# jeffreychou777/GenComm

Measured on AMD Instinct MI355X. Metric: scenes/sec, higher is better.
Workload: dtype f32

## Files before the change

### gencomm_amd/csrc/gencomm_abi.hip

```cpp
#include "../../include/gencomm_hip.h"

#include "common.h"
#include "conv_kernels.h"
#include "detect_kernels.h"
#include "enhancer_host.h"
#include "fusion_kernels.h"
#include "msgext_host.h"
#include "noise_kernels.h"
#include "pillar_kernels.h"
#include "pfn_kernels.h"
#include "train_kernels.h"
#include "wgrad_h3_kernels.h"
#include "unet_bwd_host.h"
#include "unet_host.h"

#include <algorithm>
#include <atomic>
#include <map>
#include <mutex>
#include <string>
#include <stdlib.h>
#include <string.h>

namespace gc {
// ... 470 lines not shown
  if (const char* e = w.build(p, n, H, W)) return fail(GC_ERR_ARG, e);
  if ((long long)w.total > workspace_bytes) return fail(GC_ERR_WORKSPACE, "workspace too small (see gencomm_denoise_workspace_bytes)");
  hipStream_t st = (hipStream_t)stream;
  const bool philox = noise0 == nullptr;
  const long long per_agent = (long long)C * H * W;

  UNetCall c{&p, &w, prepared, (char*)workspace, n, H, W, st, modes_snapshot()};
  if (int rc = check_bf16_mode(c.m, p, W)) return rc;
  GC_HIP(hipMemsetAsync(c.amax(), 0, 256, st));
  amax_kernel<<<256, 256, 0, st>>>(cond, (long long)n * 2 * H * W, c.amax());
  QSampleArgs q{feat, src_row, noise0, sched + (size_t)(T - 1) * 5, out, seed, (unsigned)T, per_agent, seed_dev, c.amax() + 1};
  launch_q_sample(q, n, philox, st);

  const long long smode = c.m.v[MODE_SAMPLER];
  const bool want_latent = smode == 2 || (smode == 0 && pick_tile(c.m, n, H, W) == TILE_64x16);
  const bool latent = want_latent && T >= 2 && (W % 4) == 0;
  if (!latent) {
    for (int i = 0; i < T; ++i) {
      const int t = T - 1 - i;
      ConvOutArgs co{};
      co.out = out;
      co.xt = out;
      co.sched = sched + (size_t)t * 5;
      co.noise = philox ? nullptr : step_noise + (size_t)i * n * per_agent;
      co.seed = seed;
      co.seed_dev = seed_dev;
      co.stream_id = (unsigned)t;
      const int post = t == 0 ? 0 : (philox ? 2 : 1);
      if (int rc = unet_enqueue(c, out, cond, t, post, co)) return rc;
    }
    return GC_OK;
  }
  const int nops = (int)p.ops.size();
  kmap_enqueue(c, cond);
  for (int i = 0; i < T; ++i) {
    const int t = T - 1 - i;
    ConvOutArgs co{};
    co.out = out;
    if (int rc = unet_enqueue_range(c, out, cond, t, 0, co, i == 0 ? 0 : 1, t == 0 ? nops : nops - 1, i != 0, i == 0)) return rc;
    if (t > 0) {
      const float* nz = philox ? nullptr : step_noise + (size_t)i * n * per_agent;
      if (int rc = latent_step_enqueue(c, sched + (size_t)t * 5, nz, seed, (unsigned)t, seed_dev)) return rc;
    }
  }
  return GC_OK;
}

int gencomm_enhancer_num_params(int C) {
  EnhancerPlan p;
  if (const char* e = p.build(C)) { fail(GC_ERR_ARG, e); return -1; }
  return (int)p.params.size();
}
int gencomm_enhancer_param_info(int C, int index, char* name, int name_cap, long long* numel, long long* offset) {
  EnhancerPlan p;
  if (const char* e = p.build(C)) return fail(GC_ERR_ARG, e);
  GC_CHECK_ARG(index >= 0 && index < (int)p.params.size(), "param index out of range");
  GC_CHECK_ARG(name && name_cap > 0 && numel && offset, "null output pointer");
  snprintf(name, (size_t)name_cap, "%s", p.params[index].name.c_str());
  *numel = p.params[index].numel;
  *offset = p.params[index].off;
  return GC_OK;
}
long long gencomm_enhancer_raw_floats(int C) {
  EnhancerPlan p;
  if (const char* e = p.build(C)) { fail(GC_ERR_ARG, e); return -1; }
  return p.raw_floats;
}
long long gencomm_enhancer_workspace_bytes(int n, int C, int H, int W) {
  EnhancerPlan p;
  if (const char* e = p.build(C)) { fail(GC_ERR_ARG, e); return -1; }
  if (n < 1 || H < 1 || W < 1) { fail(GC_ERR_ARG, "n, H, W must be positive"); return -1; }
  return (long long)enhancer_workspace_bytes(p, n, H, W);
// ... 614 lines not shown
```

### gencomm_amd/csrc/latent_kernels.h

```cpp
#pragma once
#include "unet_kernels.h"

namespace gc {

struct PrepLatentArgs {
  const float* w_in;
  const float* w_out;
  const float* b_out;
  float* wc5; float* wc1; float* bring; float* bsum;
  int C;
};
__global__ void prep_latent_kernel(const PrepLatentArgs a) {
  const int idx = blockIdx.x * blockDim.x + threadIdx.x;
  const int C = a.C, CI = C + 2;
  auto Wx = [&](int o, int c, int t) { return (double)a.w_in[((size_t)o * CI + 2 + c) * 9 + t]; };
  auto Wo = [&](int c, int i, int t) { return (double)a.w_out[((size_t)c * 8 + i) * 9 + t]; };
  if (idx < 1600) {
    const int o = idx & 7, d = (idx >> 3) % 25, i = idx / 200;
    const int dy = d / 5, dx = d % 5;
    double s = 0.0;
    for (int t1y = 0; t1y < 3; ++t1y)
      for (int t1x = 0; t1x < 3; ++t1x) {
        const int t2y = dy - t1y, t2x = dx - t1x;
        if (t2y < 0 || t2y > 2 || t2x < 0 || t2x > 2) continue;
// ... 10 lines not shown
    const int j = idx - 1600 - 5184, o = j & 7, t1 = j >> 3;
    double s = 0.0;
    for (int c = 0; c < C; ++c) s += Wx(o, c, t1) * (double)a.b_out[c];
    a.bring[j] = (float)s;
  } else if (idx < 1600 + 5184 + 72 + 8) {
    const int o = idx - 1600 - 5184 - 72;
    double s = 0.0;
    for (int t1 = 0; t1 < 9; ++t1)
      for (int c = 0; c < C; ++c) s += Wx(o, c, t1) * (double)a.b_out[c];
    a.bsum[o] = (float)s;
  }
}

struct LatentArgs {
  const float* a_src;
  const double* a_stat;
  const float* gamma; const float* beta;
  const float* kmap;
  float* hs0;
  double* hs0_stat;
  const float* wc5; const float* wc1; const float* bring; const float* bsum;
  const float* wx;
  const float* wc5h;
  const float* wxh;
  const float* noise;
  const float* sched;
  double inv_cnt;
  unsigned long long seed;
  unsigned int stream_id;
  int C, H, W;
  const unsigned long long* seed_dev;
  int xcd;
  int a_bf16;
};

template <int TW, int TH, int NOISE>
__global__ __launch_bounds__((TW / 4) * TH) void latent_step_kernel(const LatentArgs a) {
  constexpr int NT = (TW / 4) * TH, QPR = TW / 4;
  constexpr int LH5 = TH + 4, LH = TH + 2, LS = TW + 8;
  static_assert(NT / QPR == TH, "one staging pass must cover TH rows");
  __shared__ __align__(16) float smem[8 * LH5 * LS];
  __shared__ float s_ab[8][2];
  __shared__ float s_red[NT / 64][16];
  float (*tileA)[LH5][LS] = reinterpret_cast<float (*)[LH5][LS]>(smem);
  float (*tileE)[LH][LS] = reinterpret_cast<float (*)[LH][LS]>(smem);

  const int tid = threadIdx.x, lane = tid & 63;
  const BlockId bid = xcd_block(a.xcd);
  const int n = bid.z;
  const int x0 = bid.x * TW, y0 = bid.y * TH;
  const int tx = tid % QPR, ty = tid / QPR;
  const int H = a.H, W = a.W;
  const unsigned plane = (unsigned)(H * W);
  const float c1 = as_const(a.sched)[2], c2 = as_const(a.sched)[3], sg = as_const(a.sched)[4];
  const unsigned long long seed = (NOISE == 2 && a.seed_dev) ? *a.seed_dev : a.seed;

  float wc[25];
  load_wregs<25>(wc, a.wc5, 1600, lane);
  const float* __restrict__ ap = a.a_src + (size_t)n * 8 * plane;
  float4 qm[8], qr[(4 * 8 * QPR + NT - 1) / NT];
  constexpr int NREM = (4 * 8 * QPR + NT - 1) / NT;
  constexpr int NHAL = (8 * LH5 * 4 + NT - 1) / NT;
  float hh[NHAL];
  auto load_quad = [&](int c, int r, int qx) {
    const int gy = y0 - 2 + r, gx = x0 + 4 * qx;
    float4 v = make_float4(0.f, 0.f, 0.f, 0.f);
    if (r < LH5 && gy >= 0 && gy < H && gx < W) v = *reinterpret_cast<const float4*>(ap + ((unsigned)c * plane + (unsigned)gy * (unsigned)W + (unsigned)gx));
    return v;
  };
#pragma unroll
  for (int c = 0; c < 8; ++c) qm[c] = load_quad(c, ty, tx);
#pragma unroll
  for (int j = 0; j < NREM; ++j) {
    const int idx = tid + j * NT;
    const int c = idx / (4 * QPR), rr = TH + (idx / QPR) % 4;
    qr[j] = c < 8 ? load_quad(c, rr, tx) : make_float4(0.f, 0.f, 0.f, 0.f);
  }
#pragma unroll
  for (int j = 0; j < NHAL; ++j) {
// ... 231 lines not shown
```

### gencomm_amd/csrc/latenth_kernels.h

```cpp
#pragma once
#include "conv8b_kernels.h"
#include "conv8h_kernels.h"
#include "latent_kernels.h"

namespace gc {

constexpr int HL_LH5 = HC_TH + 4;
constexpr int HL_PLANE5 = HL_LH5 * HC_ROW;
constexpr int HL_W5TAB3 = 8 * HC_WC3;
constexpr int HL_TPLANE5 = HL_PLANE5 / 2;
constexpr int HL_RING = (2 * (HC_TW + 4) + 2 * HL_LH5) * 8;

__global__ __launch_bounds__(256) void prep_latent_h_kernel(const float* __restrict__ wc5, const float* __restrict__ w_in ,
                                                           float* __restrict__ dst5, float* __restrict__ dstx,
                                                           float* __restrict__ dstc, int C) {
  __shared__ float s_max[256];
  const int tid = threadIdx.x;
  const int CI = C + 2;
  float m = 0.f;
  for (int i = tid; i < 1600; i += 256) m = fmaxf(m, fabsf(wc5[i]));
  for (int i = tid; i < 8 * CI * 9; i += 256) m = fmaxf(m, fabsf(w_in[i]));
  s_max[tid] = m;
  __syncthreads();
  for (int s = 128; s > 0; s >>= 1) {
// ... 103 lines not shown
      const float* __restrict__ w = a.wc1 + (t1 * 9 + t2) * 64;
#pragma unroll 2
      for (int i = 0; i < 8; ++i) {
        float av[4];
#pragma unroll
        for (int p = 0; p < 4; ++p) {
          const int tr = trow + t1y + t2y, tp = px0 + p + t1x + t2x - 2;
          av[p] = inp[p] ? ring[hl_ring_slot(y0 - 2 + tr, x0 + tp, tr, tp, H, W) * 8 + i] : 0.f;
        }
#pragma unroll
        for (int o = 0; o < 4; ++o) {
          const float wv = w[i * 8 + oc0 + o] * sc;
#pragma unroll
          for (int p = 0; p < 4; ++p) accp[p][o] = fmaf(-wv, av[p], accp[p][o]);
        }
      }
    }
  }
}


struct ConvInHArgs {
  const float* cond;
  const float* x;
  const float* wch;
  const float* wxh;
  const float* scales;
  const float* bias;
  float* dst;
  double* dstat;
  int C, H, W;
  int xcd;
  const float* amax;
};

__global__ __launch_bounds__(HC_NT, 3) void conv_in_h_kernel(const ConvInHArgs a) {
  constexpr int NT = HC_NT, TW = HC_TW, TH = HC_TH;
  __shared__ __align__(16) unsigned char tile[2 * HC_PLANE + HC_TPLANE];
  __shared__ float s_red[NT / 64][16];
  fp16_ovfl_clamp();
  const int tid = threadIdx.x, lane = tid & 63, wave = tid >> 6;
  const BlockId bid = xcd_block(a.xcd);
  const int n = bid.z;
  const int x0 = bid.x * TW, y0 = bid.y * TH;
  const int H = a.H, W = a.W;
  const unsigned plane = (unsigned)(H * W);
  const int ln = lane & 15, g = lane >> 4, ch = g & 1, rr = g >> 1;
  const int gx = x0 + 4 * ln, gy0 = y0 + 4 * wave + rr;
  const bool wave_live = y0 + 4 * wave < H;
  const int r0 = tid >> 4, qx = tid & 15;
  const float mul = a.amax != nullptr ? act_scale(fmaxf(a.amax[0], a.C > 0 ? a.amax[1] : 0.f)) : 1.0f;
  const float inv_s = a.scales[0] / mul, sc = a.scales[1] * mul;

  f32x4 acc[2][4];
  {
    const float4 b4 = *reinterpret_cast<const float4*>(a.bias + 4 * ch);
    const f32x4 b0 = {b4.x * sc, b4.y * sc, b4.z * sc, b4.w * sc};
#pragma unroll
    for (int p = 0; p < 2; ++p)
#pragma unroll
      for (int j = 0; j < 4; ++j) acc[p][j] = b0;
  }
  int off[4][3];
  hc_lane_offsets(off, wave, lane);
  const int nchunk = a.C / 8;
  const float* __restrict__ xp = a.x + (size_t)n * a.C * plane;
  TileRegs<TW, TH, NT, 8> R;
  float2 hreg = make_float2(0.f, 0.f);
  {
    const float* __restrict__ sp = a.cond + (size_t)n * 2 * plane;
    TileRegs<TW, TH, NT, 2> Rc;
    stage_load<TW, TH, NT, 2, false>(Rc, sp, plane, W, H, W, x0, y0, tid);
    float2 hc = make_float2(0.f, 0.f);
    if (tid < HC_LH * 8 && (tid & 3) == 0) {
      const int side = (tid >> 2) & 1, r = tid >> 3;
      const int gy = y0 - 1 + r, gxh = side ? x0 + TW : x0 - 1;
      if (gy >= 0 && gy < H && gxh >= 0 && gxh < W) {
        hc.x = sp[(unsigned)gy * (unsigned)W + (unsigned)gxh];
        hc.y = sp[plane + (unsigned)gy * (unsigned)W + (unsigned)gxh];
      }
    }
    if (nchunk > 0) {
      stage_load<TW, TH, NT, 8, false>(R, xp, plane, W, H, W, x0, y0, tid);
      hreg = halo_load_h<false>(xp, plane, W, H, W, x0, y0, tid);
    }
    float e[8][4];
#pragma unroll
    for (int c = 0; c < 8; ++c)
#pragma unroll
      for (int j = 0; j < 4; ++j) e[c][j] = 0.f;
    e[0][0] = Rc.v[0].x * mul; e[0][1] = Rc.v[0].y * mul; e[0][2] = Rc.v[0].z * mul; e[0][3] = Rc.v[0].w * mul;
    e[1][0] = Rc.v[1].x * mul; e[1][1] = Rc.v[1].y * mul; e[1][2] = Rc.v[1].z * mul; e[1][3] = Rc.v[1].w * mul;
    hc_store_main3(tile, r0, qx, e);
    const float er[4] = {Rc.vr.x * mul, Rc.vr.y * mul, Rc.vr.z * mul, Rc.vr.w * mul};
    hc_store_rem3(tile, tid, er);
    if (tid < HC_LH * 8) hc_store_halo3(tile, tid, hc.x * mul, hc.y * mul);
    __syncthreads();
    if (wave_live) conv_tile_mfma3<false, true>(tile, a.wch, acc, off, lane);
  }
#pragma unroll 1
  for (int cc = 0; cc < nchunk; ++cc) {
    __syncthreads();
    stage_store_h<false, true>(tile, R, hreg, H, W, x0, y0, nullptr, tid, mul);
    if (cc + 1 < nchunk) {
      stage_load<TW, TH, NT, 8, false>(R, xp + (size_t)(cc + 1) * 8 * plane, plane, W, H, W, x0, y0, tid);
      hreg = halo_load_h<false>(xp + (size_t)(cc + 1) * 8 * plane, plane, W, H, W, x0, y0, tid);
    }
    __syncthreads();
    if (wave_live) conv_tile_mfma3<false, true>(tile, a.wxh + (size_t)cc * HC_WTAB3, acc, off, lane);
  }

  float part[8];
#pragma unroll
  for (int i = 0; i < 8; ++i) part[i] = 0.f;
  if (wave_live) {
#pragma unroll
    for (int p = 0; p < 2; ++p) {
      const int gy = gy0 + 2 * p;
      if (gy < H && gx + 3 < W) {
#pragma unroll
        for (int i = 0; i < 4; ++i) {
          float v[4];
#pragma unroll
          for (int j = 0; j < 4; ++j) {
            v[j] = acc[p][j][i] * inv_s;
            part[i] += v[j];
            part[4 + i] = fmaf(v[j], v[j], part[4 + i]);
          }
          *reinterpret_cast<float4*>(a.dst + ((size_t)n * 8 + 4 * ch + i) * plane + (size_t)gy * W + gx) = make_float4(v[0], v[1], v[2], v[3]);
        }
      }
// ... 163 lines not shown
            if (POST != 0) {
              const float4 t4 = *reinterpret_cast<const float4*>(a.xt + e);
              const float xt[4] = {t4.x, t4.y, t4.z, t4.w};
              if (POST == 1) {
                const float4 z4 = *reinterpret_cast<const float4*>(a.noise + e);
                const float z[4] = {z4.x, z4.y, z4.z, z4.w};
#pragma unroll
                for (int j = 0; j < 4; ++j) v[j] = fmaf(sg, z[j], fmaf(c1, v[j], c2 * xt[j]));
              } else {
#pragma unroll
                for (int j = 0; j < 4; ++j) v[j] = z8[4 * ii + j] + fmaf(c1, v[j], c2 * xt[j]);
              }
            }
            *reinterpret_cast<float4*>(a.out + e) = make_float4(v[0], v[1], v[2], v[3]);
            if (POST != 0) amax = fmaxf(amax, fmaxf(fmaxf(fabsf(v[0]), fabsf(v[1])), fmaxf(fabsf(v[2]), fabsf(v[3]))));
          }
        }
      }
    }
  }
  if (POST != 0 && a.amax_out != nullptr) wave_amax_commit(amax, a.amax_out);
}

template <int NOISE>
__global__ __launch_bounds__(HC_NT, 3) void latent_step_h_kernel(const LatentArgs a) {
  constexpr int NT = HC_NT, TW = HC_TW, TH = HC_TH;
  constexpr int TILE_BYTES = NOISE == 1 ? 2 * HC_PLANE + HC_TPLANE : 2 * HL_PLANE5;
  __shared__ __align__(16) unsigned char tile[TILE_BYTES];
  __shared__ float s_ring[HL_RING];
  __shared__ float s_ab[8][2];
  __shared__ float s_red[NT / 64][16];

  fp16_ovfl_clamp();
  const int tid = threadIdx.x, lane = tid & 63, wave = tid >> 6;
  const BlockId bid = xcd_block(a.xcd);
  const int n = bid.z;
  const int x0 = bid.x * TW, y0 = bid.y * TH;
  const int H = a.H, W = a.W;
  const unsigned plane = (unsigned)(H * W);
  const float c1 = a.sched[2], c2 = a.sched[3], sg = a.sched[4];
  const unsigned long long seed = (NOISE == 2 && a.seed_dev) ? *a.seed_dev : a.seed;
  const int ln = lane & 15, g = lane >> 4, ch = g & 1, rr = g >> 1;
  const int gx = x0 + 4 * ln;
  const int gy0 = y0 + 4 * wave + rr;
  const bool wave_live = y0 + 4 * wave < H;

  const int af32 = !a.a_bf16;
  const size_t abase = (size_t)n * 8 * plane;
  float4 qm[8], qr[2];
  float hh[2][2];
  const int r0 = tid >> 4, qx = tid & 15;
  const bool ok_m = (y0 - 2 + r0) >= 0 && (y0 - 2 + r0) < H && (x0 + 4 * qx) < W;
#pragma unroll
  for (int c = 0; c < 8; ++c)
    qm[c] = ok_m ? ld4(a.a_src, af32, abase + ((unsigned)c * plane + (unsigned)(y0 - 2 + r0) * (unsigned)W + (unsigned)(x0 + 4 * qx)))
                 : make_float4(0.f, 0.f, 0.f, 0.f);
  const int rrow = TH + ((tid & 63) >> 4), cpr = tid >> 6;
  const bool ok_r = (y0 - 2 + rrow) >= 0 && (y0 - 2 + rrow) < H && (x0 + 4 * qx) < W;
#pragma unroll
  for (int k = 0; k < 2; ++k)
    qr[k] = ok_r ? ld4(a.a_src, af32, abase + ((unsigned)(2 * cpr + k) * plane + (unsigned)(y0 - 2 + rrow) * (unsigned)W + (unsigned)(x0 + 4 * qx)))
                 : make_float4(0.f, 0.f, 0.f, 0.f);
  bool ok_h[2];
#pragma unroll
  for (int j = 0; j < 2; ++j) {
    const int idx = tid + j * NT;
// ... 283 lines not shown
```

### gencomm_amd/csrc/unet_host.h

```cpp
#pragma once
#include <stdlib.h>

#include "attn_kernels.h"
#include "conv8b_kernels.h"
#include "conv8h_kernels.h"
#include "conv8h8_kernels.h"
#include "dataflow_kernels.h"
#include "latent_kernels.h"
#include "latenth_kernels.h"
#include "unet_kernels.h"
#include "unet_plan.h"

namespace gc {

inline int cdiv(int a, int b) { return (a + b - 1) / b; }

enum TileCfg { TILE_64x16 = 0, TILE_32x16 = 1, TILE_32x8 = 2 };
inline long long tile_want(const Modes& m) {
  return m.v[MODE_TILE_WANT] > 0 ? m.v[MODE_TILE_WANT] : (m.split() ? 160LL : 512LL);
}
inline TileCfg pick_tile(const Modes& m, int n, int H, int W, int zmul = 1) {
  if (m.bf16()) return TILE_64x16;
  const long long want = tile_want(m);
  if ((long long)cdiv(W, 64) * cdiv(H, 16) * n * zmul >= want) return TILE_64x16;
// ... 51 lines not shown
  }
  GC_KLOG(t == TILE_64x16 ? "conv8_kernel<64,16,4,...> (exact fp32)" : t == TILE_32x16 ? "conv8_kernel<32,16,4,...> (exact fp32)" : "conv8_kernel<32,8,1,...> (exact fp32)");
  switch (t) {
    case TILE_64x16: conv8_kernel<64, 16, 4, NSRC, GN, UP, RES><<<grid, 256, 0, st>>>(a); break;
    case TILE_32x16: conv8_kernel<32, 16, 4, NSRC, GN, UP, RES><<<grid, 128, 0, st>>>(a); break;
    default: conv8_kernel<32, 8, 1, NSRC, GN, UP, RES><<<grid, 256, 0, st>>>(a); break;
  }
}

template <int NSRC, bool GN, bool UP, int RES>
inline void launch_conv8b(const Conv8BArgs& a, int n, hipStream_t st) {
  const double elt = 2.0;
  const double abytes = elt * n * ((double)NSRC * 8 * a.Hin * a.Win + (RES == 1 ? 8.0 : RES == 2 ? 16.0 : 0.0) * a.H * a.W + 8.0 * a.H * a.W);
  TimedLaunch tl(UP ? KF_UP : (NSRC == 2 ? KF_CONV16 : (RES == 1 ? KF_CONV8_RES1 : RES == 2 ? KF_CONV8_RES2 : KF_CONV8)), st, abytes);
  GC_KLOG("conv8b_kernel<...> (bf16 storage)");
  conv8b_kernel<NSRC, GN, UP, RES><<<dim3(cdiv(a.W, 64), cdiv(a.H, 16), n), 256, 0, st>>>(a);
}

struct UNetCall {
  const UNetPlan* plan;
  const UNetWorkspace* ws;
  const float* prepared;
  char* wsp;
  int n, H, W;
  hipStream_t st;
  Modes m;
  float* amax() const { return reinterpret_cast<float*>(wsp + ws->amax_off); }
  int is_f32(int id) const { return (!m.bf16() || id == plan->hs0_tensor) ? 1 : 0; }

  float* tensor_ptr(int id) const {
    const TensorPlan& t = plan->tensors[id];
    return reinterpret_cast<float*>(wsp + ws->level_base[t.level] + ws->slot_bytes[t.level] * t.slot);
  }
  double* stat_ptr(int id) const { return reinterpret_cast<double*>(wsp) + (size_t)id * n * 16; }
};

inline Conv8Args conv1_args(const UNetCall& c, const Op& o, int t) {
  const ResBlockPlan& b = c.plan->blocks[o.blk];
  const float* P = c.prepared;
  const int Hl = c.ws->Hl[o.level], Wl = c.ws->Wl[o.level];
  Conv8Args a{};
  a.src[0] = c.tensor_ptr(o.src[0]); a.sstat[0] = c.stat_ptr(o.src[0]);
  if (o.src[1] >= 0) { a.src[1] = c.tensor_ptr(o.src[1]); a.sstat[1] = c.stat_ptr(o.src[1]); }
  a.gamma = P + b.n1w; a.beta = P + b.n1b;
  a.w = P + b.p_c1w; a.wh = P + b.p_c1wh; a.bias = P + b.p_bias1 + (size_t)t * 8;
  a.dst = c.tensor_ptr(o.dst); a.dstat = c.stat_ptr(o.dst);
  a.H = a.Hin = Hl; a.W = a.Win = Wl;
  a.inv_cnt = 1.0 / ((b.cin == 8 ? 2.0 : 4.0) * Hl * Wl);
  a.xcd = c.m.xcd();
  return a;
}
inline Conv8Args conv2_args(const UNetCall& c, const Op& o) {
  const ResBlockPlan& b = c.plan->blocks[o.blk];
  const float* P = c.prepared;
  const int Hl = c.ws->Hl[o.level], Wl = c.ws->Wl[o.level];
  Conv8Args a{};
  a.src[0] = c.tensor_ptr(o.src[0]); a.sstat[0] = c.stat_ptr(o.src[0]);
  a.gamma = P + b.n2w; a.beta = P + b.n2b;
  a.w = P + b.p_c2w; a.wh = P + b.p_c2wh; a.bias = P + b.p_bias2;
  a.res[0] = c.tensor_ptr(o.res[0]);
  if (o.res[1] >= 0) { a.res[1] = c.tensor_ptr(o.res[1]); a.ninw = P + b.p_ninw; }
  a.dst = c.tensor_ptr(o.dst); a.dstat = c.stat_ptr(o.dst);
  a.H = a.Hin = Hl; a.W = a.Win = Wl;
  a.inv_cnt = 1.0 / (2.0 * Hl * Wl);
  a.xcd = c.m.xcd();
  return a;
}
// ... 4 lines not shown
  Conv8Args a{};
  a.src[0] = c.tensor_ptr(o.src[0]);
  a.sstat[0] = c.stat_ptr(o.src[0]);
  a.w = P + p.up[lin].p_w; a.wh = P + p.up[lin].p_wh; a.bias = P + p.up[lin].b;
  a.dst = c.tensor_ptr(o.dst); a.dstat = c.stat_ptr(o.dst);
  a.H = c.ws->Hl[o.level]; a.W = c.ws->Wl[o.level]; a.Hin = c.ws->Hl[lin]; a.Win = c.ws->Wl[lin];
  a.xcd = c.m.xcd();
  return a;
}
inline DownArgs down_args(const UNetCall& c, const Op& o) {
  const UNetPlan& p = *c.plan;
  const float* P = c.prepared;
  const int lin = o.level - 1;
  return DownArgs{c.tensor_ptr(o.src[0]), P + p.down[lin].p_w, P + p.down[lin].b, c.tensor_ptr(o.dst), c.stat_ptr(o.dst),
                  c.ws->Hl[o.level], c.ws->Wl[o.level], c.ws->Hl[lin], c.ws->Wl[lin], !c.is_f32(o.src[0]), !c.is_f32(o.dst)};
}

inline bool resfuse_emulated(const UNetCall& c, const ResBlockPlan& b, TileCfg tc, bool wvec) {
  return c.m.v[MODE_RESFUSE_EMU] != 0 && b.cin == 8 && tc == TILE_64x16 && c.m.split() && !c.m.bf16() && wvec;
}

inline bool df_eligible(const UNetCall& c, int f, int l) {
  if (c.m.v[MODE_DATAFLOW] == 0 || !c.m.split() || c.m.bf16() || l - f < 2 || l - f > DF_MAX_OPS || c.n > 64 * 1024) return false;
  if (c.m.v[MODE_CONV8H_MASK] != -1) return false;
  for (int oi = f; oi < l; ++oi) {
    const Op& o = c.plan->ops[oi];
    if (o.kind != OP_RES_CONV1 && o.kind != OP_RES_CONV2 && o.kind != OP_DOWN && o.kind != OP_UP) return false;
    if (o.kind == OP_DOWN) {
      if ((c.ws->Wl[o.level - 1] & 3) != 0) return false;
    } else if (pick_tile(c.m, c.n, c.ws->Hl[o.level], c.ws->Wl[o.level]) != TILE_64x16) return false;
  }
  return true;
}
inline int df_enqueue(const UNetCall& c, int t, int f, int l, bool upload) {
  const UNetPlan& p = *c.plan;
  DfProgram* dprog = reinterpret_cast<DfProgram*>(c.wsp + c.ws->df_prog_off);
  unsigned* words = reinterpret_cast<unsigned*>(c.wsp + c.ws->df_words_off);
  const int nops = l - f;
  if (upload) {
    static thread_local DfProgram hp;
    hp.nops = nops; hp.n = c.n;
    int qlen[8] = {0, 0, 0, 0, 0, 0, 0, 0};
    for (int k = 0; k < nops; ++k) {
      const Op& o = p.ops[f + k];
      DfOp& d = hp.ops[k];
      d = DfOp{};
      const int Hl = c.ws->Hl[o.level], Wl = c.ws->Wl[o.level];
      if (o.kind == OP_DOWN) {
        d.kind = DF_DOWN; d.tx = cdiv(Hl * ((Wl + 1) / 2), 256); d.ty = 1; d.down = down_args(c, o);
      } else {
        d.tx = cdiv(Wl, 64); d.ty = cdiv(Hl, 16);
        if (o.kind == OP_RES_CONV1) {
          d.kind = p.blocks[o.blk].cin == 8 ? DF_CONV1 : DF_CONV16; d.conv = conv1_args(c, o, 0); d.bias_stride = 8;
        } else if (o.kind == OP_RES_CONV2) {
          d.kind = p.blocks[o.blk].cin == 8 ? DF_CONV2_RES1 : DF_CONV2_RES2; d.conv = conv2_args(c, o);
        } else {
          d.kind = DF_UP; d.conv = up_args(c, o);
        }
      }
      d.tiles = d.tx * d.ty;
      d.items = d.tiles * c.n;
      const int qq = d.items >> 3, rr = d.items & 7;
      for (int x = 0; x <= 8; ++x) d.item_base[x] = x * qq + (x < rr ? x : rr);
      for (int x = 0; x < 8; ++x) { d.ticket_base[x] = qlen[x]; qlen[x] += d.item_base[x + 1] - d.item_base[x]; }
    }
    for (int x = 0; x < 8; ++x) hp.queue_len[x] = qlen[x];
    for (int k0 = 0; k0 < nops; k0 += DF_CHUNK) {
      DfUploadArgs ua{};
      ua.dst = dprog; ua.first = k0; ua.count = std::min(DF_CHUNK, nops - k0); ua.nops = nops; ua.n = c.n;
      for (int x = 0; x < 8; ++x) ua.queue_len[x] = qlen[x];
      for (int k = 0; k < ua.count; ++k) ua.ops[k] = hp.ops[k0 + k];
      df_upload_kernel<<<1, 64, 0, c.st>>>(ua);
    }
  }
  int dev = 0, cus = 256;
  if (hipGetDevice(&dev) == hipSuccess) (void)hipDeviceGetAttribute(&cus, hipDeviceAttributeMultiprocessorCount, dev);
  DfArgs da{dprog, words, words + 8, words + 8 + 64 * (size_t)c.n, t, c.m.v[MODE_DATAFLOW] == 2 ? 1 : 0};
  GC_KLOG("unet_dataflow_kernel (persistent, per-agent layer dependencies)");
  TimedLaunch tl(KF_DATAFLOW, c.st);
  unet_dataflow_kernel<<<dim3(3 * cus), HC_NT, 0, c.st>>>(da);
  GC_HIP(hipGetLastError());
  return GC_OK;
}

inline int unet_enqueue_range(const UNetCall& c, const float* x_t, const float* cond, int t, int post,
                              ConvOutArgs co, int first, int last, bool keep_hs0_stats, bool df_upload = true) {
  const UNetPlan& p = *c.plan;
  const float* P = c.prepared;
  {
    const size_t skip = keep_hs0_stats ? (size_t)c.n * 16 * sizeof(double) : 0;
    GC_HIP(hipMemsetAsync(c.wsp + skip, 0, c.ws->stats_bytes - skip, c.st));
  }
  const int df_f = std::max(first, 1), df_l = std::min(last, (int)p.ops.size() - 1);
  const bool dataflow = df_eligible(c, df_f, df_l);
  for (int oi = first; oi < last; ++oi) {
    if (dataflow && oi == df_f) {
      if (int rc = df_enqueue(c, t, df_f, df_l, df_upload)) return rc;
      oi = df_l - 1;
      continue;
    }
    const Op& o = p.ops[oi];
    const int Hl = c.ws->Hl[o.level], Wl = c.ws->Wl[o.level];
    switch (o.kind) {
      case OP_CONV_IN: {
        ConvInArgs a{cond, x_t, P + p.conv_in.p_w, P + p.conv_in.b, c.tensor_ptr(o.dst), c.stat_ptr(o.dst), p.C, Hl, Wl, c.m.xcd()};
        const TileCfg tc = pick_tile(c.m, c.n, Hl, Wl);
        int tw, th;
        tile_dims(tc, &tw, &th);
        const dim3 grid(cdiv(Wl, tw), cdiv(Hl, th), c.n);
        TimedLaunch tl(KF_CONV_IN, c.st);
        if (tc == TILE_64x16 && c.m.split() && (Wl & 3) == 0) {
          ConvInHArgs ah{cond, x_t, P + p.p_wch, P + p.p_wxh, P + p.p_wc5h + HL_W5TAB3, P + p.conv_in.b, c.tensor_ptr(o.dst),
                         c.stat_ptr(o.dst), p.C, Hl, Wl, c.m.xcd(), c.amax()};
          GC_KLOG("conv_in_h_kernel");
          conv_in_h_kernel<<<grid, 256, 0, c.st>>>(ah);
        } else {
          GC_KLOG("conv_in_kernel<tile> (exact fp32)");
          if (tc == TILE_64x16) conv_in_kernel<64, 16, 4><<<grid, 256, 0, c.st>>>(a);
          else if (tc == TILE_32x16) conv_in_kernel<32, 16, 4><<<grid, 128, 0, c.st>>>(a);
          else conv_in_kernel<32, 8, 1><<<grid, 256, 0, c.st>>>(a);
        }
        break;
      }
      case OP_RES_CONV1: {
        const ResBlockPlan& b = p.blocks[o.blk];
        if (c.m.bf16()) {
          Conv8BArgs a{};
          a.src[0] = c.tensor_ptr(o.src[0]); a.src_f32[0] = c.is_f32(o.src[0]); a.sstat[0] = c.stat_ptr(o.src[0]);
          if (o.src[1] >= 0) { a.src[1] = c.tensor_ptr(o.src[1]); a.src_f32[1] = c.is_f32(o.src[1]); a.sstat[1] = c.stat_ptr(o.src[1]); }
          a.gamma = P + b.n1w; a.beta = P + b.n1b; a.wb = P + b.p_c1wb; a.bias = P + b.p_bias1 + (size_t)t * 8;
          a.dst = c.tensor_ptr(o.dst); a.dst_f32 = c.is_f32(o.dst); a.dstat = c.stat_ptr(o.dst);
          a.H = a.Hin = Hl; a.W = a.Win = Wl; a.inv_cnt = 1.0 / ((b.cin == 8 ? 2.0 : 4.0) * Hl * Wl); a.xcd = c.m.xcd();
          if (b.cin == 8) launch_conv8b<1, true, false, 0>(a, c.n, c.st);
          else launch_conv8b<2, true, false, 0>(a, c.n, c.st);
          break;
        }
        const Conv8Args a = conv1_args(c, o, t);
        const TileCfg tc = pick_tile(c.m, c.n, Hl, Wl);
        if (resfuse_emulated(c, b, tc, (Wl & 3) == 0)) {
          Conv8Args e = a;
          e.term_mask = 63 | 64;
          TimedLaunch tl(KF_CONV8, c.st, 4.0 * c.n * 8.0 * Hl * Wl);
          GC_KLOG("conv8h_kernel<1,GN,0,0,DIAG> (MODE_RESFUSE_EMU: statistics only)");
          conv8h_kernel<1, true, false, 0, true><<<dim3(cdiv(Wl, 64), cdiv(Hl, 16), c.n), 256, 0, c.st>>>(e);
          break;
        }
// ... 80 lines not shown
        tile_dims(tc, &tw, &th);
        const dim3 grid(cdiv(Wl, tw), cdiv(Hl, th), c.n * nocb);
#define GC_LAUNCH_CO(POST)                                                             \
  do {                                                                                 \
    if (tc == TILE_64x16) conv_out_kernel<64, 16, 4, POST><<<grid, 256, 0, c.st>>>(co); \
    else conv_out_kernel<32, 8, 1, POST><<<grid, 256, 0, c.st>>>(co);                  \
  } while (0)
        TimedLaunch tl(KF_CONV_OUT, c.st);
        if (c.m.split() && (Wl & 3) == 0 && pick_tile(c.m, c.n, Hl, Wl) == TILE_64x16) {
          const dim3 gh(cdiv(Wl, 64), cdiv(Hl, 16), c.n);
          GC_KLOG(post == 0 ? "conv_out_h_kernel<0> (x0_hat)" : post == 1 ? "conv_out_h_kernel<1> (explicit noise)" : "conv_out_h_kernel<2> (in-kernel Philox)");
          if (post == 0) conv_out_h_kernel<0><<<gh, 256, 0, c.st>>>(co);
          else if (post == 1) conv_out_h_kernel<1><<<gh, 256, 0, c.st>>>(co);
          else conv_out_h_kernel<2><<<gh, 256, 0, c.st>>>(co);
        } else {
          GC_KLOG(post == 0 ? "conv_out_kernel<tile,0> (exact fp32, x0_hat)" : post == 1 ? "conv_out_kernel<tile,1> (exact fp32, explicit noise)" : "conv_out_kernel<tile,2> (exact fp32, in-kernel Philox)");
          if (post == 0) GC_LAUNCH_CO(0);
          else if (post == 1) GC_LAUNCH_CO(1);
          else GC_LAUNCH_CO(2);
        }
#undef GC_LAUNCH_CO
        break;
      }
    }
  }
  GC_HIP(hipGetLastError());
  return GC_OK;
}

inline int unet_enqueue(const UNetCall& c, const float* x_t, const float* cond, int t, int post, ConvOutArgs co) {
  return unet_enqueue_range(c, x_t, cond, t, post, co, 0, (int)c.plan->ops.size(), false);
}

inline void kmap_enqueue(const UNetCall& c, const float* cond) {
  const UNetPlan& p = *c.plan;
  ConvInArgs a{cond, nullptr, c.prepared + p.conv_in.p_w, c.prepared + p.conv_in.b,
               reinterpret_cast<float*>(c.wsp + c.ws->kmap_off), nullptr, 0, c.H, c.W, c.m.xcd()};
  const TileCfg tc = pick_tile(c.m, c.n, c.H, c.W);
  int tw, th;
  tile_dims(tc, &tw, &th);
  const dim3 grid(cdiv(c.W, tw), cdiv(c.H, th), c.n);
  if (tc == TILE_64x16 && c.m.split() && (c.W & 3) == 0) {
    ConvInHArgs ah{cond, nullptr, c.prepared + p.p_wch, c.prepared + p.p_wxh, c.prepared + p.p_wc5h + HL_W5TAB3, c.prepared + p.conv_in.b,
                   reinterpret_cast<float*>(c.wsp + c.ws->kmap_off), nullptr, 0, c.H, c.W, c.m.xcd(), c.amax()};
    conv_in_h_kernel<<<grid, 256, 0, c.st>>>(ah);
  } else if (tc == TILE_64x16) conv_in_kernel<64, 16, 4><<<grid, 256, 0, c.st>>>(a);
  else if (tc == TILE_32x16) conv_in_kernel<32, 16, 4><<<grid, 128, 0, c.st>>>(a);
  else conv_in_kernel<32, 8, 1><<<grid, 256, 0, c.st>>>(a);
}

inline int latent_step_enqueue(const UNetCall& c, const float* sched_row, const float* noise, unsigned long long seed,
                               unsigned stream_id, const unsigned long long* seed_dev = nullptr) {
  const UNetPlan& p = *c.plan;
  const float* P = c.prepared;
  GC_HIP(hipMemsetAsync(c.stat_ptr(p.hs0_tensor), 0, (size_t)c.n * 16 * sizeof(double), c.st));
  LatentArgs a{};
  a.a_src = c.tensor_ptr(p.last_body_tensor); a.a_stat = c.stat_ptr(p.last_body_tensor);
  a.gamma = P + p.nout_w; a.beta = P + p.nout_b;
  a.kmap = reinterpret_cast<const float*>(c.wsp + c.ws->kmap_off);
  a.hs0 = c.tensor_ptr(p.hs0_tensor); a.hs0_stat = c.stat_ptr(p.hs0_tensor);
  a.wc5 = P + p.p_wc5; a.wc1 = P + p.p_wc1; a.bring = P + p.p_bring; a.bsum = P + p.p_bsum;
  a.wx = P + p.conv_in.p_w + 144;
  a.wc5h = P + p.p_wc5h; a.wxh = P + p.p_wxh;
  a.noise = noise; a.sched = sched_row; a.inv_cnt = 1.0 / (2.0 * c.H * c.W);
  a.seed = seed; a.seed_dev = seed_dev; a.stream_id = stream_id; a.C = p.C; a.H = c.H; a.W = c.W;
  a.xcd = c.m.xcd();
  a.a_bf16 = !c.is_f32(p.last_body_tensor);
  TimedLaunch tl(KF_LATENT_STEP, c.st, 4.0 * c.n * 32.0 * c.H * c.W);
  const bool small_h = c.m.split() && (c.W & 3) == 0 && c.W >= 64 && c.H >= 16 && c.m.v[MODE_TILE_WANT] == 0;
  if ((pick_tile(c.m, c.n, c.H, c.W) == TILE_64x16 || small_h) && c.m.split()) {
    const dim3 grid(cdiv(c.W, 64), cdiv(c.H, 16), c.n);
    GC_KLOG(noise ? "latent_step_h_kernel<1> (explicit noise)" : "latent_step_h_kernel<2> (in-kernel Philox)");
    if (noise) latent_step_h_kernel<1><<<grid, 256, 0, c.st>>>(a);
    else latent_step_h_kernel<2><<<grid, 256, 0, c.st>>>(a);
  } else if (pick_tile(c.m, c.n, c.H, c.W) == TILE_64x16) {
    const dim3 grid(cdiv(c.W, 64), cdiv(c.H, 16), c.n);
    GC_KLOG(noise ? "latent_step_kernel<64,16,1> (exact fp32, explicit noise)" : "latent_step_kernel<64,16,2> (exact fp32, in-kernel Philox)");
    if (noise) latent_step_kernel<64, 16, 1><<<grid, 256, 0, c.st>>>(a);
    else latent_step_kernel<64, 16, 2><<<grid, 256, 0, c.st>>>(a);
  } else {
    const dim3 grid(cdiv(c.W, 32), cdiv(c.H, 16), c.n);
    GC_KLOG(noise ? "latent_step_kernel<32,16,1> (exact fp32, explicit noise)" : "latent_step_kernel<32,16,2> (exact fp32, in-kernel Philox)");
    if (noise) latent_step_kernel<32, 16, 1><<<grid, 128, 0, c.st>>>(a);
    else latent_step_kernel<32, 16, 2><<<grid, 128, 0, c.st>>>(a);
  }
  GC_HIP(hipGetLastError());
  return GC_OK;
}

inline int unet_prepare_enqueue(const UNetPlan& p, const float* raw, float* prepared, hipStream_t st) {
  GC_HIP(hipMemcpyAsync(prepared, raw, (size_t)p.raw_floats * sizeof(float), hipMemcpyDeviceToDevice, st));
  auto conv_w = [&](long long src, long long dst, int OC, int IC, int OCB) {
    const int total = OC * IC * 9;
    prep_conv_w_kernel<<<cdiv(total, 256), 256, 0, st>>>(raw + src, prepared + dst, OC, IC, OCB);
// ... 43 lines not shown
```

### gencomm_amd/csrc/unet_plan.h

```cpp
#pragma once
#include <string>
#include <vector>

#include "common.h"

namespace gc {

constexpr int kWtab3 = 3 * (3 * 64 * 4 + 64 * 2);

struct ParamEntry {
  std::string name;
  long long numel;
  long long off;
};

struct ResBlockPlan {
  int cin;
  long long n1w, n1b, c1w, c1b, tpw, tpb, n2w, n2b, c2w, c2b, ninw, ninb;
  long long p_c1w, p_c2w, p_ninw, p_bias1 , p_bias2 ;
  long long p_c1wh, p_c2wh;
  long long p_c1wb, p_c2wb;
};

struct AttnPlan {
// ... 218 lines not shown
    tensors[hs0_tensor].last_use = (int)ops.size();
    slots_per_level.assign(L, 0);
    std::vector<std::vector<int>> free_slots(L);
    auto take_slot = [&](int id) {
      TensorPlan& t = tensors[id];
      if (!free_slots[t.level].empty()) {
        t.slot = free_slots[t.level].back();
        free_slots[t.level].pop_back();
      } else {
        t.slot = slots_per_level[t.level]++;
      }
    };
    for (int i = 0; i < (int)ops.size(); ++i) {
      const Op& o = ops[i];
      if (o.kind == OP_ATTN) { take_slot(o.src[1]); take_slot(o.res[0]); take_slot(o.res[1]); }
      if (o.dst >= 0) take_slot(o.dst);
      for (int k = 0; k < 4; ++k) {
        const int id = k < 2 ? o.src[k] : o.res[k - 2];
        if (id >= 0 && tensors[id].last_use == i && tensors[id].slot >= 0) {
          bool dup = false;
          for (int k2 = 0; k2 < k; ++k2) dup |= ((k2 < 2 ? o.src[k2] : o.res[k2 - 2]) == id);
          if (!dup && !keep_all) free_slots[tensors[id].level].push_back(tensors[id].slot);
        }
      }
    }
    return nullptr;
  }
};

struct UNetWorkspace {
  std::vector<int> Hl, Wl;
  std::vector<size_t> level_base, slot_bytes;
  size_t stats_bytes = 0, total = 0, kmap_off = 0, amax_off = 0;
  size_t df_words_off = 0, df_prog_off = 0;

  const char* build(const UNetPlan& p, int n, int H, int W) {
    Hl.assign(p.L, 0); Wl.assign(p.L, 0);
    Hl[0] = H; Wl[0] = W;
    for (int l = 1; l < p.L; ++l) {
      if ((Hl[l - 1] & 1) || (Wl[l - 1] & 1)) return "H and W must be even at every level that is downsampled";
      Hl[l] = Hl[l - 1] / 2; Wl[l] = Wl[l - 1] / 2;
    }
    if (Hl[p.L - 1] < 1 || Wl[p.L - 1] < 1) return "feature map too small for the number of levels";
    df_words_off = align_up(p.tensors.size() * (size_t)n * 16 * sizeof(double), 256);
    stats_bytes = align_up(df_words_off + (8 + 64 * (size_t)n + 4) * sizeof(unsigned), 256);
    size_t off = stats_bytes;
    level_base.assign(p.L, 0); slot_bytes.assign(p.L, 0);
    for (int l = 0; l < p.L; ++l) {
      slot_bytes[l] = align_up((size_t)n * 8 * Hl[l] * Wl[l] * sizeof(float), 256);
      level_base[l] = off;
      off += slot_bytes[l] * p.slots_per_level[l];
    }
    kmap_off = off;
    off += slot_bytes[0];
    amax_off = off;
    off += 256;
    df_prog_off = off;
    off += 1 << 16;
    total = off;
    return nullptr;
  }
};

}
```

Baseline: 185.7.

## Fold stats clearing into latent step and emit kmap from first conv_in

Removes the per-step hipMemsetAsync calls for normalization statistics. The latent step kernel now zeroes the stats area, using double-buffered (parity) stat slots for the hs0 and last-body tensors so the slots it reads and accumulates are not cleared. It also drops the separate kmap conv_in launch by having the first step's conv_in_h kernel write the message-only partial result as the kmap. The cost is extra stores in the kernels and more complex slot bookkeeping. The dataflow program is now uploaded on every step.

```diff
diff --git a/gencomm_amd/csrc/gencomm_abi.hip b/gencomm_amd/csrc/gencomm_abi.hip
--- a/gencomm_amd/csrc/gencomm_abi.hip
+++ b/gencomm_amd/csrc/gencomm_abi.hip
@@ -526,12 +526,17 @@
     return GC_OK;
   }
   const int nops = (int)p.ops.size();
-  kmap_enqueue(c, cond);
+  GC_HIP(hipMemsetAsync(c.wsp, 0, w.stats_bytes, st));
+  float* kmap_out = nullptr;
+  if (kmap_from_conv_in(c)) kmap_out = reinterpret_cast<float*>(c.wsp + w.kmap_off);
+  else kmap_enqueue(c, cond);
   for (int i = 0; i < T; ++i) {
     const int t = T - 1 - i;
+    c.alt = i & 1;
     ConvOutArgs co{};
     co.out = out;
-    if (int rc = unet_enqueue_range(c, out, cond, t, 0, co, i == 0 ? 0 : 1, t == 0 ? nops : nops - 1, i != 0, i == 0)) return rc;
+    if (int rc = unet_enqueue_range(c, out, cond, t, 0, co, i == 0 ? 0 : 1, t == 0 ? nops : nops - 1, true,
+                                    i == 0 ? kmap_out : nullptr)) return rc;
     if (t > 0) {
       const float* nz = philox ? nullptr : step_noise + (size_t)i * n * per_agent;
       if (int rc = latent_step_enqueue(c, sched + (size_t)t * 5, nz, seed, (unsigned)t, seed_dev)) return rc;
diff --git a/gencomm_amd/csrc/latent_kernels.h b/gencomm_amd/csrc/latent_kernels.h
--- a/gencomm_amd/csrc/latent_kernels.h
+++ b/gencomm_amd/csrc/latent_kernels.h
@@ -66,7 +66,19 @@
   const unsigned long long* seed_dev;
   int xcd;
   int a_bf16;
+  double* clr;
+  int clr_count, clr_len, clr_keep0, clr_keep1;
 };
+
+__device__ __forceinline__ void latent_clear_stats(const LatentArgs& a, int nt) {
+  if (a.clr == nullptr) return;
+  const unsigned long long wg = blockIdx.x + (unsigned long long)gridDim.x * (blockIdx.y + (unsigned long long)gridDim.y * blockIdx.z);
+  const unsigned long long stride = (unsigned long long)gridDim.x * gridDim.y * gridDim.z * (unsigned)nt;
+  for (unsigned long long i = wg * (unsigned)nt + threadIdx.x; i < (unsigned long long)a.clr_count; i += stride) {
+    const unsigned j = (unsigned)i;
+    if (j - (unsigned)a.clr_keep0 >= (unsigned)a.clr_len && j - (unsigned)a.clr_keep1 >= (unsigned)a.clr_len) a.clr[j] = 0.0;
+  }
+}
 
 template <int TW, int TH, int NOISE>
 __global__ __launch_bounds__((TW / 4) * TH) void latent_step_kernel(const LatentArgs a) {
@@ -79,6 +91,7 @@
   float (*tileA)[LH5][LS] = reinterpret_cast<float (*)[LH5][LS]>(smem);
   float (*tileE)[LH][LS] = reinterpret_cast<float (*)[LH][LS]>(smem);
 
+  latent_clear_stats(a, NT);
   const int tid = threadIdx.x, lane = tid & 63;
   const BlockId bid = xcd_block(a.xcd);
   const int n = bid.z;
diff --git a/gencomm_amd/csrc/latenth_kernels.h b/gencomm_amd/csrc/latenth_kernels.h
--- a/gencomm_amd/csrc/latenth_kernels.h
+++ b/gencomm_amd/csrc/latenth_kernels.h
@@ -159,6 +159,7 @@
   int C, H, W;
   int xcd;
   const float* amax;
+  float* kmap;
 };
 
 __global__ __launch_bounds__(HC_NT, 3) void conv_in_h_kernel(const ConvInHArgs a) {
@@ -224,6 +225,18 @@
     if (tid < HC_LH * 8) hc_store_halo3(tile, tid, hc.x * mul, hc.y * mul);
     __syncthreads();
     if (wave_live) conv_tile_mfma3<false, true>(tile, a.wch, acc, off, lane);
+    if (a.kmap != nullptr && wave_live) {
+#pragma unroll
+      for (int p = 0; p < 2; ++p) {
+        const int gy = gy0 + 2 * p;
+        if (gy < H && gx + 3 < W) {
+#pragma unroll
+          for (int i = 0; i < 4; ++i)
+            *reinterpret_cast<float4*>(a.kmap + ((size_t)n * 8 + 4 * ch + i) * plane + (size_t)gy * W + gx) =
+                make_float4(acc[p][0][i] * inv_s, acc[p][1][i] * inv_s, acc[p][2][i] * inv_s, acc[p][3][i] * inv_s);
+        }
+      }
+    }
   }
 #pragma unroll 1
   for (int cc = 0; cc < nchunk; ++cc) {
@@ -453,6 +466,7 @@
   __shared__ float s_red[NT / 64][16];
 
   fp16_ovfl_clamp();
+  latent_clear_stats(a, NT);
   const int tid = threadIdx.x, lane = tid & 63, wave = tid >> 6;
   const BlockId bid = xcd_block(a.xcd);
   const int n = bid.z;
diff --git a/gencomm_amd/csrc/unet_host.h b/gencomm_amd/csrc/unet_host.h
--- a/gencomm_amd/csrc/unet_host.h
+++ b/gencomm_amd/csrc/unet_host.h
@@ -107,7 +107,15 @@
     const TensorPlan& t = plan->tensors[id];
     return reinterpret_cast<float*>(wsp + ws->level_base[t.level] + ws->slot_bytes[t.level] * t.slot);
   }
-  double* stat_ptr(int id) const { return reinterpret_cast<double*>(wsp) + (size_t)id * n * 16; }
+  int alt = 0;
+
+  double* stat_slot(int slot) const { return reinterpret_cast<double*>(wsp) + (size_t)slot * n * 16; }
+  int stat_slot_of(int id, int parity) const {
+    if (parity && id == plan->hs0_tensor) return ws->stat_slots - 2;
+    if (parity && id == plan->last_body_tensor) return ws->stat_slots - 1;
+    return id;
+  }
+  double* stat_ptr(int id) const { return stat_slot(stat_slot_of(id, alt)); }
 };
 
 inline Conv8Args conv1_args(const UNetCall& c, const Op& o, int t) {
@@ -178,12 +186,12 @@
   }
   return true;
 }
-inline int df_enqueue(const UNetCall& c, int t, int f, int l, bool upload) {
+inline int df_enqueue(const UNetCall& c, int t, int f, int l) {
   const UNetPlan& p = *c.plan;
   DfProgram* dprog = reinterpret_cast<DfProgram*>(c.wsp + c.ws->df_prog_off);
   unsigned* words = reinterpret_cast<unsigned*>(c.wsp + c.ws->df_words_off);
   const int nops = l - f;
-  if (upload) {
+  {
     static thread_local DfProgram hp;
     hp.nops = nops; hp.n = c.n;
     int qlen[8] = {0, 0, 0, 0, 0, 0, 0, 0};
@@ -230,18 +238,16 @@
 }
 
 inline int unet_enqueue_range(const UNetCall& c, const float* x_t, const float* cond, int t, int post,
-                              ConvOutArgs co, int first, int last, bool keep_hs0_stats, bool df_upload = true) {
+                              ConvOutArgs co, int first, int last, bool stats_ready, float* kmap_out = nullptr) {
   const UNetPlan& p = *c.plan;
   const float* P = c.prepared;
-  {
-    const size_t skip = keep_hs0_stats ? (size_t)c.n * 16 * sizeof(double) : 0;
-    GC_HIP(hipMemsetAsync(c.wsp + skip, 0, c.ws->stats_bytes - skip, c.st));
-  }
   const int df_f = std::max(first, 1), df_l = std::min(last, (int)p.ops.size() - 1);
   const bool dataflow = df_eligible(c, df_f, df_l);
+  if (!stats_ready) GC_HIP(hipMemsetAsync(c.wsp, 0, c.ws->stats_bytes, c.st));
+  else if (dataflow) GC_HIP(hipMemsetAsync(c.wsp + c.ws->df_words_off, 0, c.ws->stats_bytes - c.ws->df_words_off, c.st));
   for (int oi = first; oi < last; ++oi) {
     if (dataflow && oi == df_f) {
-      if (int rc = df_enqueue(c, t, df_f, df_l, df_upload)) return rc;
+      if (int rc = df_enqueue(c, t, df_f, df_l)) return rc;
       oi = df_l - 1;
       continue;
     }
@@ -257,7 +263,7 @@
         TimedLaunch tl(KF_CONV_IN, c.st);
         if (tc == TILE_64x16 && c.m.split() && (Wl & 3) == 0) {
           ConvInHArgs ah{cond, x_t, P + p.p_wch, P + p.p_wxh, P + p.p_wc5h + HL_W5TAB3, P + p.conv_in.b, c.tensor_ptr(o.dst),
-                         c.stat_ptr(o.dst), p.C, Hl, Wl, c.m.xcd(), c.amax()};
+                         c.stat_ptr(o.dst), p.C, Hl, Wl, c.m.xcd(), c.amax(), kmap_out};
           GC_KLOG("conv_in_h_kernel");
           conv_in_h_kernel<<<grid, 256, 0, c.st>>>(ah);
         } else {
@@ -404,6 +410,9 @@
   return unet_enqueue_range(c, x_t, cond, t, post, co, 0, (int)c.plan->ops.size(), false);
 }
 
+inline bool kmap_from_conv_in(const UNetCall& c) {
+  return pick_tile(c.m, c.n, c.H, c.W) == TILE_64x16 && c.m.split() && (c.W & 3) == 0;
+}
 inline void kmap_enqueue(const UNetCall& c, const float* cond) {
   const UNetPlan& p = *c.plan;
   ConvInArgs a{cond, nullptr, c.prepared + p.conv_in.p_w, c.prepared + p.conv_in.b,
@@ -412,6 +421,7 @@
   int tw, th;
   tile_dims(tc, &tw, &th);
   const dim3 grid(cdiv(c.W, tw), cdiv(c.H, th), c.n);
+  GC_KLOG("k map (conv_in on the message channels alone)");
   if (tc == TILE_64x16 && c.m.split() && (c.W & 3) == 0) {
     ConvInHArgs ah{cond, nullptr, c.prepared + p.p_wch, c.prepared + p.p_wxh, c.prepared + p.p_wc5h + HL_W5TAB3, c.prepared + p.conv_in.b,
                    reinterpret_cast<float*>(c.wsp + c.ws->kmap_off), nullptr, 0, c.H, c.W, c.m.xcd(), c.amax()};
@@ -425,13 +435,18 @@
                                unsigned stream_id, const unsigned long long* seed_dev = nullptr) {
   const UNetPlan& p = *c.plan;
   const float* P = c.prepared;
-  GC_HIP(hipMemsetAsync(c.stat_ptr(p.hs0_tensor), 0, (size_t)c.n * 16 * sizeof(double), c.st));
   LatentArgs a{};
   a.a_src = c.tensor_ptr(p.last_body_tensor); a.a_stat = c.stat_ptr(p.last_body_tensor);
+  const int keep_read = c.stat_slot_of(p.last_body_tensor, c.alt), keep_acc = c.stat_slot_of(p.hs0_tensor, c.alt ^ 1);
+  a.clr = c.stat_slot(0);
+  a.clr_count = c.ws->stat_slots * c.n * 16;
+  a.clr_len = c.n * 16;
+  a.clr_keep0 = keep_read * c.n * 16;
+  a.clr_keep1 = keep_acc * c.n * 16;
   a.gamma = P + p.nout_w; a.beta = P + p.nout_b;
   a.kmap = reinterpret_cast<const float*>(c.wsp + c.ws->kmap_off);
-  a.hs0 = c.tensor_ptr(p.hs0_tensor); a.hs0_stat = c.stat_ptr(p.hs0_tensor);
-  a.wc5 = P + p.p_wc5; a.wc1 = P + p.p_wc1; a.bring = P + p.p_bring; a.bsum = P + p.p_bsum;
+  a.hs0 = c.tensor_ptr(p.hs0_tensor); a.hs0_stat = c.stat_slot(keep_acc);
+  a.wc5 =P + p.p_wc5; a.wc1 = P + p.p_wc1; a.bring = P + p.p_bring; a.bsum = P + p.p_bsum;
   a.wx = P + p.conv_in.p_w + 144;
   a.wc5h = P + p.p_wc5h; a.wxh = P + p.p_wxh;
   a.noise = noise; a.sched = sched_row; a.inv_cnt = 1.0 / (2.0 * c.H * c.W);
diff --git a/gencomm_amd/csrc/unet_plan.h b/gencomm_amd/csrc/unet_plan.h
--- a/gencomm_amd/csrc/unet_plan.h
+++ b/gencomm_amd/csrc/unet_plan.h
@@ -274,6 +274,7 @@
   std::vector<int> Hl, Wl;
   std::vector<size_t> level_base, slot_bytes;
   size_t stats_bytes = 0, total = 0, kmap_off = 0, amax_off = 0;
+  int stat_slots = 0;
   size_t df_words_off = 0, df_prog_off = 0;
 
   const char* build(const UNetPlan& p, int n, int H, int W) {
@@ -284,7 +285,8 @@
       Hl[l] = Hl[l - 1] / 2; Wl[l] = Wl[l - 1] / 2;
     }
     if (Hl[p.L - 1] < 1 || Wl[p.L - 1] < 1) return "feature map too small for the number of levels";
-    df_words_off = align_up(p.tensors.size() * (size_t)n * 16 * sizeof(double), 256);
+    stat_slots = (int)p.tensors.size() + 2;
+    df_words_off = align_up((size_t)stat_slots * n * 16 * sizeof(double), 256);
     stats_bytes = align_up(df_words_off + (8 + 64 * (size_t)n + 4) * sizeof(unsigned), 256);
     size_t off = stats_bytes;
     level_base.assign(p.L, 0); slot_bytes.assign(p.L, 0);
```

Result: no change. 185.9, median of 6 (+0.1%).
